# Daaohame/RAHT-3DGS-codec

Hardware: AMD Instinct MI355X
Metric: M-Gaussians/s fwd+inv RAHT, 59-ch SH3 3DGS (higher is better)
Workload: dtype f32 (xyz columns: f64); 1 GPU; cfg3: 2999072 Gaussians (3000000 draws/GPU, J=12, 59 channels), fwd RAHT + quantize/reorder + dequantize/un-reorder + inv RAHT (quantization fused into the transform kernels); the 3 xyz columns carried in float64 inside the same launches (raht_fwd_quant_mixed / raht_dequant_inv_mixed): the reference's integers on every column; rows_per_gpu=2999072, channels=59, depth_J=12, engine=tile, quantize=True, parallelism=1 GPU, world=1

## Files before the change

### raht-3dgs-codec_amd/csrc/schedule.hip

```cpp
#include "raht_common.h"

#include <algorithm>
#include <atomic>

namespace raht {

__global__ void compact_scatter_kernel(const uint32_t *in, const uint32_t *flag, const uint32_t *pos, uint32_t *out, int64_t n);

__global__ void stage_survivor_kernel(const uint32_t *__restrict__ rows, int64_t n, int R, int64_t N,
                                      const int32_t *__restrict__ wl, const int32_t *__restrict__ wr,
                                      const uint8_t *__restrict__ lvl, int top_level,
                                      uint32_t *__restrict__ survivor)
{
    const int64_t j = (int64_t)blockIdx.x * blockDim.x + threadIdx.x;
    if (j >= n) return;
    const int64_t r = rows ? rows[j] : j;
    const int64_t t = j / R;
    const int64_t j0 = t * R, j1 = j0 + R;
    const int64_t start = rows ? rows[j0] : j0;
    const int64_t end = (j1 < n) ? (rows ? (int64_t)rows[j1] : j1) : N;
    const bool merged = (r > 0) && ((int)lvl[r] < top_level) && (r - wl[r] >= start) && (r + wr[r] <= end);
    survivor[j] = merged ? 0u : 1u;
}

// ... 398 lines not shown
                                   const int64_t *__restrict__ wsum, int top_level, uint32_t *__restrict__ pj,
                                   double *__restrict__ ab, uint8_t *__restrict__ bucket, uint32_t *__restrict__ is_root)
{
    const int64_t e = (int64_t)blockIdx.x * blockDim.x + threadIdx.x;
    if (e >= n) return;
    const int64_t r = rows ? (int64_t)rows[e] : e;
    const int l = (int)lvl[r];
    const bool merged = (r > 0) && (l < top_level);
    is_root[e] = merged ? 0u : 1u;
    bucket[e] = merged ? (uint8_t)l : (uint8_t)63;
    uint32_t rec = 0;
    double a = 0.0, b = 0.0;
    if (merged) {
        const int64_t want = r - wl[r];
        int64_t p = want;
        if (rows) {
            int64_t lo = 0, hi = e - 1;
            while (lo < hi) {
                const int64_t mid = (lo + hi) >> 1;
                if ((int64_t)rows[mid] < want) lo = mid + 1; else hi = mid;
            }
            p = lo;
        }
        double w0, w1;
        pair_weights(r, wl[r], wr[r], wsum, w0, w1);
        const double den = w0 + w1;
        a = sqrt(w0 / den);
        b = sqrt(w1 / den);
        rec = (uint32_t)p | ((uint32_t)e << 16);
    }
    pj[e] = rec; ab[2 * e] = a; ab[2 * e + 1] = b;
}

__global__ void top_gather_kernel(const uint32_t *__restrict__ perm, uint32_t n_merges, const uint32_t *__restrict__ pj,
                                  const double *__restrict__ ab, uint32_t *__restrict__ t_pj,
                                  float *__restrict__ t_ab32, double *__restrict__ t_ab64)
{
    const uint32_t k = blockIdx.x * blockDim.x + threadIdx.x;
    if (k >= n_merges) return;
    const uint32_t e = perm[k];
    t_pj[k] = pj[e];
    const double a = ab[2 * e], b = ab[2 * e + 1];
    t_ab64[2 * k] = a; t_ab64[2 * k + 1] = b;
    t_ab32[2 * k] = (float)a; t_ab32[2 * k + 1] = (float)b;
}

__global__ void top_root_rank_kernel(const uint32_t *__restrict__ is_root, const uint32_t *__restrict__ pos, int64_t n,
                                     uint32_t *__restrict__ t_root)
{
    const int64_t e = (int64_t)blockIdx.x * blockDim.x + threadIdx.x;
    if (e < n) t_root[e] = is_root[e] ? pos[e] : 0xffffffffu;
}

static hipError_t gather_stage_meta(const raht_plan *plan, Stage &st, hipStream_t s)
{
    const size_t n = (size_t)st.n_entries;
    hipError_t e = hipSuccess;
    if ((e = st.e_wl.alloc(n)) != hipSuccess || (e = st.e_wr.alloc(n)) != hipSuccess || (e = st.e_lvl.alloc(n)) != hipSuccess ||
        (e = st.e_pos.alloc(n)) != hipSuccess) return e;
    hipLaunchKernelGGL(gather_meta_kernel, dim3((unsigned)ceil_div((int64_t)n, 256)), dim3(256), 0, s, st.rows, (int64_t)n, plan->wl,
                       plan->wr, plan->lvl, plan->inv_order, st.e_wl, st.e_wr, st.e_lvl, st.e_pos);
    return hipSuccess;
}

static int build_top_stage(raht_plan *plan, int64_t n, hipStream_t s, Stage &st)
{
    st.is_top = true;
    st.n_entries = n;
    st.n_tiles = 1;
    st.tile_rows = (int)n;
    const uint32_t *rows = st.rows;
    const unsigned gb = (unsigned)ceil_div(n, 256);
    if (rows) RAHT_HIP_CHECK(gather_stage_meta(plan, st, s));
    Scratch buf(sizeof(double) * 2 * (size_t)n + sizeof(uint32_t) * (4 * (size_t)n + 66) + (size_t)n, s);
    if (!buf.ok()) return RAHT_ERR_NOMEM;
    double *ab = buf.as<double>();
    uint32_t *pj = (uint32_t *)(ab + 2 * n), *is_root = pj + n, *pos = is_root + n, *perm = pos + n, *boff = perm + n,
             *total = boff + 65;
    uint8_t *bucket = (uint8_t *)(total + 1);
    hipLaunchKernelGGL(top_resolve_kernel, dim3(gb), dim3(256), 0, s, rows, n, plan->wl, plan->wr, plan->lvl, plan->wsum,
                       plan->top_level, pj, ab, bucket, is_root);
    RAHT_RET(exclusive_scan_u32(is_root, pos, n, total, s));
    RAHT_HIP_CHECK(st.t_root.alloc((size_t)n));
    hipLaunchKernelGGL(top_root_rank_kernel, dim3(gb), dim3(256), 0, s, is_root, pos, n, st.t_root);
    RAHT_RET(bucket_sort_u8(bucket, perm, n, 6, boff, s));
    RAHT_RET(read_back_u32(st.t_loff, boff, 65, nullptr, nullptr, 0, s));
    st.n_merges = st.t_loff[63];
    {
        uint32_t *lev = st.t_lev_host;
        int nlev = 0;
        for (int l = 0; l < 63; ++l)
            if (st.t_loff[l + 1] > st.t_loff[l]) { lev[2 * nlev] = st.t_loff[l]; lev[2 * nlev + 1] = st.t_loff[l + 1]; ++nlev; }
        int nbig = nlev;
        while (nbig > 0 && lev[2 * (nbig - 1) + 1] - lev[2 * (nbig - 1)] <= 64) --nbig;
        const size_t lds_budget = 160 * 1024 - 1024;
        while (nbig < nlev && (size_t)n * 16 + (size_t)(st.n_merges - lev[2 * nbig]) * 20 > lds_budget) ++nbig;
        st.t_nlev = nlev; st.t_nbig = nbig;
        st.t_small_start = (nbig < nlev) ? lev[2 * nbig] : st.n_merges;
        RAHT_HIP_CHECK(st.t_lev.alloc(2 * 64));
        RAHT_HIP_CHECK(hipMemcpyAsync(st.t_lev, lev, sizeof(uint32_t) * 2 * (size_t)std::max(nlev, 1), hipMemcpyHostToDevice, s));
    }
    const size_t nm = std::max<size_t>(st.n_merges, 1);
    RAHT_HIP_CHECK(st.t_pj.alloc(nm));
    RAHT_HIP_CHECK(st.t_ab32.alloc(2 * nm));
    RAHT_HIP_CHECK(st.t_ab64.alloc(2 * nm));
    if (st.n_merges)
        hipLaunchKernelGGL(top_gather_kernel, dim3((unsigned)ceil_div(st.n_merges, 256)), dim3(256), 0, s, perm, st.n_merges,
                           pj, ab, st.t_pj, st.t_ab32, st.t_ab64);
    return RAHT_OK;
}

constexpr int SB_THREADS = 256, SB_ITEMS = 8, SB_BLOCK = SB_THREADS * SB_ITEMS;
constexpr int SCHED_SPEC_MAX = 8;
enum { SK_NONE = 0, SK_TILE = 1, SK_TOP = 2 };

struct SchedState {
    uint32_t n[SCHED_SPEC_MAX + 2];
    uint32_t kind[SCHED_SPEC_MAX + 2];
    uint32_t finished;
    uint32_t last_stage, last_is_top;
    uint32_t trouble;
    uint32_t top[4];
};
constexpr int SCHED_STATE_WORDS = sizeof(SchedState) / 4;

__device__ __forceinline__ uint32_t block_sum_256(uint32_t v, uint32_t *red )
{
#pragma unroll
    for (int d = 32; d >= 1; d >>= 1) v += __shfl_xor(v, d, 64);
    if ((threadIdx.x & 63) == 0) red[threadIdx.x >> 6] = v;
    __syncthreads();
    const uint32_t t = red[0] + red[1] + red[2] + red[3];
    __syncthreads();
    return t;
// ... 107 lines not shown
#pragma unroll
        for (int q = 0; q < SB_ITEMS; ++q) { f[q] = (base + q < n) ? flags[base + q] : 0; mine += f[q]; }
    }
    uint32_t inc = mine;
    const int lane = threadIdx.x & 63, wid = threadIdx.x >> 6;
#pragma unroll
    for (int d = 1; d < 64; d <<= 1) { const uint32_t t = __shfl_up(inc, d, 64); if (lane >= d) inc += t; }
    if (lane == 63) wsum[wid] = inc;
    __syncthreads();
    uint32_t before = 0, block_tot = 0;
#pragma unroll
    for (int w = 0; w < 4; ++w) { if (w < wid) before += wsum[w]; block_tot += wsum[w]; }
    uint32_t pos = block_base + before + inc - mine;
    uint32_t tile = (uint32_t)base / (uint32_t)R;
    uint32_t next_start = tile * (uint32_t)R;
    if (next_start < (uint32_t)base) { ++tile; next_start += (uint32_t)R; }
    uint32_t g_r[SB_ITEMS], g_pos[SB_ITEMS], g_inv[SB_ITEMS];
    int32_t g_wl[SB_ITEMS], g_wr[SB_ITEMS];
    uint8_t g_lv[SB_ITEMS];
    bool keep[SB_ITEMS];
#pragma unroll
    for (int q = 0; q < SB_ITEMS; ++q) {
        const int64_t j = base + q;
        keep[q] = false; g_pos[q] = 0; g_r[q] = (uint32_t)j;
        if (j < n) {
            if ((uint32_t)j == next_start) { surv_off[tile] = pos; ++tile; next_start += (uint32_t)R; }
            if (f[q]) {
                keep[q] = pos < cap_next;
                g_pos[q] = pos;
                if (keep[q] && rows) g_r[q] = rows[j];
                ++pos;
            }
        }
    }
#pragma unroll
    for (int q = 0; q < SB_ITEMS; ++q) {
        g_wl[q] = 0; g_wr[q] = 0; g_lv[q] = 0; g_inv[q] = 0;
        if (keep[q]) { const uint32_t r = g_r[q]; g_wl[q] = p_wl[r]; g_wr[q] = p_wr[r]; g_lv[q] = p_lvl[r]; g_inv[q] = p_inv[r]; }
    }
#pragma unroll
    for (int q = 0; q < SB_ITEMS; ++q)
        if (keep[q]) { const uint32_t o = g_pos[q]; n_rows[o] = g_r[q]; n_wl[o] = g_wl[q]; n_wr[o] = g_wr[q]; n_lvl[o] = g_lv[q]; n_pos[o] = g_inv[q]; }
    if ((int64_t)blockIdx.x == nblk - 1 && threadIdx.x == 0) {
        const uint32_t total = block_base + block_tot;
        surv_off[(n + R - 1) / R] = total;
        S->n[k + 1] = total;
        if (total > cap_next) S->trouble = 1;
        else if (total == n_roots) { S->finished = 1; S->last_stage = (uint32_t)k; S->last_is_top = 0; }
        else if (total >= (uint32_t)n) S->trouble = 2;
        else S->kind[k + 1] = (total <= Rf) ? SK_TOP : SK_TILE;
    }
}

constexpr int ST_THREADS = 1024;
struct SchedTopOut { uint32_t *t_pj; float *t_ab32; double *t_ab64; uint32_t *t_root; uint32_t *t_lev; };

__device__ __forceinline__ void sched_top_body(SchedState *__restrict__ S, int k, int n, const uint32_t *__restrict__ rows,
                                               const int32_t *__restrict__ p_wl, const int32_t *__restrict__ p_wr,
                                               const uint8_t *__restrict__ p_lvl, const int64_t *__restrict__ wsum,
                                               int top_level, const SchedTopOut &O)
{
    __shared__ uint32_t s_rows[RAHT_TOP_MAX_ROWS];
    __shared__ uint32_t hist[64], cursor[64], wtot[ST_THREADS / 64];
    __shared__ uint32_t root_base;
    uint32_t *__restrict__ t_pj = O.t_pj, *__restrict__ t_root = O.t_root, *__restrict__ t_lev = O.t_lev;
    float *__restrict__ t_ab32 = O.t_ab32;
    double *__restrict__ t_ab64 = O.t_ab64;
    const int tid = threadIdx.x, lane = tid & 63, wid = tid >> 6;
    if (tid < 64) hist[tid] = 0;
    if (tid == 0) root_base = 0;
    for (int e = tid; e < n; e += ST_THREADS) s_rows[e] = rows ? rows[e] : (uint32_t)e;
    __syncthreads();
    PL_STAMP(2, 0, 8);
    for (int e0 = 0; e0 < n; e0 += ST_THREADS) {
        const int e = e0 + tid;
        bool root = false;
        if (e < n) {
            const uint32_t r = s_rows[e];
            const int l = (int)p_lvl[r];
            const bool merged = (r > 0) && (l < top_level);
            root = !merged;
            if (merged) atomicAdd(&hist[l], 1u);
        }
        const uint64_t bal = __ballot(root);
        if (lane == 0) wtot[wid] = (uint32_t)__popcll(bal);
        __syncthreads();
        uint32_t before = root_base;
        for (int w = 0; w < wid; ++w) before += wtot[w];
        if (e < n) t_root[e] = root ? before + (uint32_t)__popcll(bal & (((uint64_t)1 << lane) - 1)) : 0xffffffffu;
        __syncthreads();
        if (tid == 0) { uint32_t t = 0; for (int w = 0; w < ST_THREADS / 64; ++w) t += wtot[w]; root_base += t; }
        __syncthreads();
    }
    PL_STAMP(2, 0, 9);
    if (wid == 0) {
        const uint32_t h = (lane < 63) ? hist[lane] : 0u;
        uint32_t inc = h;
#pragma unroll
        for (int d = 1; d < 64; d <<= 1) { const uint32_t t = __shfl_up(inc, d, 64); if (lane >= d) inc += t; }
        const uint32_t first = inc - h;
        cursor[lane] = first;
        const uint32_t n_merges = (uint32_t)__shfl((int)inc, 63, 64);
        const uint64_t nonempty = __ballot(h > 0), below = ((uint64_t)1 << lane) - 1;
        const int nlev = __popcll(nonempty);
        const int my = __popcll(nonempty & below);
        if (h > 0) { t_lev[2 * my] = first; t_lev[2 * my + 1] = first + h; }
        const uint64_t big = __ballot(h > 64);
        int nbig = big ? __popcll(nonempty & (((uint64_t)2 << (63 - __clzll((long long)big))) - 1)) : 0;
        const size_t lds_budget = 160 * 1024 - 1024;
        uint32_t small_start = n_merges;
        for (;;) {
            uint32_t cand = n_merges;
            if (nbig < nlev) {
                const uint64_t owner = __ballot(h > 0 && my == nbig);
                cand = (uint32_t)__shfl((int)first, __ffsll((unsigned long long)owner) - 1, 64);
            }
            if (nbig < nlev && (size_t)n * 16 + (size_t)(n_merges - cand) * 20 > lds_budget) { ++nbig; continue; }
            small_start = cand;
            break;
        }
        if (lane == 0) {
            S->top[0] = n_merges; S->top[1] = (uint32_t)nlev; S->top[2] = (uint32_t)nbig; S->top[3] = small_start;
            S->finished = 1; S->last_stage = (uint32_t)k; S->last_is_top = 1;
        }
    }
    __syncthreads();
    PL_STAMP(2, 0, 10);
    for (int e = tid; e < n; e += ST_THREADS) {
        const uint32_t r = s_rows[e];
        const int l = (int)p_lvl[r];
        if (!((r > 0) && (l < top_level))) continue;
        const int32_t wlr = p_wl[r], wrr = p_wr[r];
        const uint32_t want = r - (uint32_t)wlr;
        int lo = 0, hi = e - 1;
        while (lo < hi) {
            const int mid = (lo + hi) >> 1;
            if (s_rows[mid] < want) lo = mid + 1; else hi = mid;
        }
        double w0, w1;
        pair_weights((int64_t)r, wlr, wrr, wsum, w0, w1);
        const double den = w0 + w1;
        const double a = sqrt(w0 / den), b = sqrt(w1 / den);
        const uint32_t pos = atomicAdd(&cursor[l], 1u);
        t_pj[pos] = (uint32_t)lo | ((uint32_t)e << 16);
        t_ab64[2 * pos] = a; t_ab64[2 * pos + 1] = b;
        t_ab32[2 * pos] = (float)a; t_ab32[2 * pos + 1] = (float)b;
    }
    PL_STAMP(2, 0, 11);
}

struct SchedStageBufs {
    uint32_t *rows[SCHED_SPEC_MAX + 2]; int32_t *wl[SCHED_SPEC_MAX + 2], *wr[SCHED_SPEC_MAX + 2];
    uint8_t *lvl[SCHED_SPEC_MAX + 2]; uint32_t *pos[SCHED_SPEC_MAX + 2], *surv[SCHED_SPEC_MAX + 2];
    uint32_t cap[SCHED_SPEC_MAX + 2];
};

__global__ __launch_bounds__(ST_THREADS) void sched_tail_kernel(SchedState *S, int k_multi, int k_last, SchedStageBufs B, int R, uint32_t Rf,
                                                                uint32_t n_roots, int64_t N, int top_level, uint32_t tail_max,
                                                                const int32_t *__restrict__ p_wl, const int32_t *__restrict__ p_wr,
                                                                const uint8_t *__restrict__ p_lvl, const uint32_t *__restrict__ p_inv,
                                                                const int64_t *__restrict__ wsum, SchedTopOut O, int64_t n_first)
{
    __shared__ uint32_t wcnt[8 * (ST_THREADS / 64)], woff[8 * (ST_THREADS / 64) + 1];
    __shared__ uint32_t s_kind[SCHED_SPEC_MAX + 2], s_n[SCHED_SPEC_MAX + 2];
    const int tid = threadIdx.x, lane = tid & 63, wid = tid >> 6;
    PL_SLOT_DECL;
    PL_STAMP_NEXT();
    if (n_first >= 0) { sched_state_init(S, (uint32_t)n_first, SK_TOP); __builtin_amdgcn_fence(__ATOMIC_RELEASE, "workgroup"); __syncthreads(); }
    if (tid < SCHED_SPEC_MAX + 2) {
        s_kind[tid] = (n_first >= 0) ? (tid == 0 ? (uint32_t)SK_TOP : (uint32_t)SK_NONE) : __atomic_load_n(&S->kind[tid], __ATOMIC_RELAXED);
        s_n[tid] = (n_first >= 0) ? (tid == 0 ? (uint32_t)n_first : 0u) : __atomic_load_n(&S->n[tid], __ATOMIC_RELAXED);
    }
    __syncthreads();
    for (int k = (k_multi == 0) ? 0 : 1; k <= k_last; ++k) {
        const uint32_t kind = s_kind[k], n = s_n[k];
        PL_STAMP_NEXT();
        if (kind == SK_TOP) {
            sched_top_body(S, k, (int)n, B.rows[k], p_wl, p_wr, p_lvl, wsum, top_level, O);
            return;
        }
        if (kind == SK_TILE && k < k_multi) continue;
        if (kind != SK_TILE || n > tail_max || n > B.cap[k] || k == k_last) return;
        const uint32_t *__restrict__ rows = B.rows[k];
        const int32_t *__restrict__ wl = B.wl[k], *__restrict__ wr = B.wr[k];
        const uint8_t *__restrict__ lvl = B.lvl[k];
        uint32_t *__restrict__ surv_off = B.surv[k];
        uint32_t *__restrict__ n_rows = B.rows[k + 1], *__restrict__ n_pos = B.pos[k + 1];
        int32_t *__restrict__ n_wl = B.wl[k + 1], *__restrict__ n_wr = B.wr[k + 1];
        uint8_t *__restrict__ n_lvl = B.lvl[k + 1];
        const uint32_t cap_next = B.cap[k + 1];
        uint32_t running = 0;
        constexpr int TI = 8, NWV = ST_THREADS / 64;
        for (uint32_t base = 0; base < n; base += ST_THREADS * TI) {
            uint32_t r[TI], e_start[TI], e_end[TI];
            int32_t e_wl[TI], e_wr[TI];
            uint8_t e_lv[TI];
            uint64_t bal[TI];
// ... 293 lines not shown
```

### raht-3dgs-codec_amd/csrc/transform_mx.hip

```cpp
#include "raht_common.h"
#include "raht_device.h"
#include "tile_engine.h"
#include "tile_host.h"

#include <algorithm>
#include <cstdlib>
#include <string>
#include <type_traits>
#include <vector>

namespace raht {

#ifdef RAHT_PHASE_CLOCKS
constexpr int MX_CLK_TILES = 4096, MX_CLK_SLOTS = 12;
__device__ unsigned long long g_phase_clk_mx[MX_CLK_TILES][MX_CLK_SLOTS];
#define MX_STAMP(k) do { if (IDENT && threadIdx.x == 0 && tile_id < MX_CLK_TILES) g_phase_clk_mx[tile_id][k] = __builtin_readcyclecounter(); } while (0)
#else
#define MX_STAMP(k) do { } while (0)
#endif

constexpr int MX_MAX_WIDE = 4;
constexpr int MX_THREADS = 512;
constexpr int MX_TOP_THREADS = 1024;
constexpr int MX_TOP_SLOTS = RAHT_TOP_MAX_ROWS / MX_TOP_THREADS;

struct StepTableMX {
    StepTable f;
    double w[MX_MAX_WIDE];
};

static size_t tile_lds_bytes_mx(int R, int NF, int nwide)
{
    const size_t data = (size_t)R * NF * 16 + (((size_t)R * nwide * 8 + 15) & ~(size_t)15);
    const size_t meta = (size_t)R * (16 + 4 + 4);
    const size_t surv = ((size_t)R * 2 + 15) & ~(size_t)15;
    return data + meta + surv;
}

struct MxPtrs {
    const double *in_w;
    double *out_w;
    double *wsn_w;
    double *root_w;
    const uint32_t *prog;
    uint32_t prog_stride, prog_ab;
    int prog_compact;
};

struct MxMultiQ {
    int k;
    uint32_t fast_div;
    double step[MULTI_Q_MAX];
    int32_t *Q[MULTI_Q_MAX];
};

template <bool INV, bool IDENT, int SLOTS, bool ROOTS, bool MULTI = false, bool SQ = false>
__device__ __forceinline__ void tile_body_mx(const TileArgs<float> &A, const MxPtrs &P, const StepTableMX &ST, const int64_t tile_id,
                                             const MxMultiQ *MQ = nullptr)
{
    extern __shared__ __align__(16) unsigned char smem[];
    typedef RegChunk<float> V16;
    typedef RegChunk<double> W16;
    typedef RegChunk<int32_t> I16;
    const int R = A.R;
    const int tid0 = threadIdx.x;
    const int nthreads = blockDim.x, nwv = nthreads >> 6;
    const int nwide = A.nwide;
    const int lgw = nwide > 2 ? 2 : nwide - 1;
    const int Df = A.D;
    const int Fp = A.Dp, NF = Fp >> 2;
    const int lg = A.lg, lr = 6 - A.lg;
// ... 533 lines not shown
__global__ __launch_bounds__(MX_THREADS, 6) void tile_kernel_mx_sq(const TileArgs<float> A, const MxPtrs P, const StepTableMX ST)
{
    tile_body_mx<true, true, SLOTS, false, false, true>(A, P, ST, (int64_t)blockIdx.x);
}

struct TileBatchMX {
    TileArgs<float> a[BATCH_MAX];
    MxPtrs p[BATCH_MAX];
    uint32_t first_tile[BATCH_MAX + 1];
    int n;
};
static_assert(sizeof(TileBatchMX) + sizeof(StepTableMX) <= 4096, "tile_kernel_mx_batch: arguments exceed the 4 KB kernarg segment");

template <bool INV, bool IDENT, int SLOTS>
__global__ __launch_bounds__(MX_THREADS, 6) void tile_kernel_mx_batch(const TileBatchMX B, const StepTableMX ST)
{
    int s = 0;
#pragma unroll
    for (int q = 1; q < BATCH_MAX; ++q) s += (q < B.n && blockIdx.x >= B.first_tile[q]) ? 1 : 0;
    tile_body_mx<INV, IDENT, SLOTS, false>(B.a[s], B.p[s], ST, (int64_t)(blockIdx.x - B.first_tile[s]));
}

struct TopArgsMX {
    const float *in_rows;  int64_t ld_in;
    const float *in_img; const double *in_img_w;
    float *out_rows;       int64_t ld_out;
    float *out_img; double *out_img_w;
    int32_t *Q;            int64_t ldq;
    const uint32_t *e_pos;
    const uint32_t *pj;
    const float *ab32;  const double *ab64;
    int n, n_merges, D, nwide, Fp;
    const uint32_t *lev;
    int nlev, nbig;
    uint32_t small_start;
    const uint32_t *root_rank;
    float *root_f; double *root_w;
};

template <bool WIDE, bool INV, bool ROOTS, bool MULTI = false>
__device__ __forceinline__ void top_body_mx(const TopArgsMX &A, const StepTableMX &ST, const int chunk, const MxMultiQ *MQ = nullptr)
{
    typedef typename std::conditional<WIDE, double, float>::type T;
    constexpr int VN = WIDE ? 2 : 4;
    typedef RegChunk<T> V16;
    extern __shared__ __align__(16) unsigned char smem[];
    V16 *tile = (V16 *)smem;
    __shared__ uint32_t s_lev[2 * 64];
    const int tid = threadIdx.x;
    const int nwide = A.nwide;
    const int goff = WIDE ? 2 * chunk : min(chunk * 4, A.D - 4);
    const int ioff = chunk * 4;
    const int n = A.n, nm = A.n_merges;
    if (tid < 2 * A.nlev) s_lev[tid] = A.lev[tid];
    const T *ab = WIDE ? (const T *)A.ab64 : (const T *)A.ab32;
    const int n_small = nm - (int)A.small_start;
    uint32_t *s_pj = (uint32_t *)(smem + (size_t)n * 16);
    T *s_ab = (T *)(s_pj + ((n_small + 3) & ~3));
    for (int i = tid; i < n_small; i += MX_TOP_THREADS) {
        s_pj[i] = A.pj[A.small_start + i];
        s_ab[2 * i] = ab[2 * (A.small_start + i)];
        s_ab[2 * i + 1] = ab[2 * (A.small_start + i) + 1];
    }
    T my_step[VN];
    float my_rcp[VN];
    bool live[VN];
#pragma unroll
    for (int i = 0; i < VN; ++i) {
        if constexpr (WIDE) { live[i] = goff + i < nwide; my_step[i] = live[i] ? ST.w[goff + i] : 1.0; my_rcp[i] = 1.0f; }
        else { live[i] = !(chunk == 0 && i < nwide); my_step[i] = ST.f.v[ST.f.n == 1 ? 0 : goff + i]; my_rcp[i] = refined_rcp(my_step[i]); }
    }
    uint32_t pj[MX_TOP_SLOTS];
    T ra[MX_TOP_SLOTS], rb[MX_TOP_SLOTS];
#pragma unroll
    for (int k = 0; k < MX_TOP_SLOTS; ++k) {
        const int idx = min(k * MX_TOP_THREADS + tid, max(nm - 1, 0));
        pj[k] = A.pj[idx]; ra[k] = ab[2 * idx]; rb[k] = ab[2 * idx + 1];
    }
    uint32_t m_dst[MX_TOP_SLOTS], m_rr[MX_TOP_SLOTS];
#pragma unroll
    for (int k = 0; k < MX_TOP_SLOTS; ++k) {
        m_dst[k] = A.e_pos[min(k * MX_TOP_THREADS + tid, n - 1)];
        m_rr[k] = ROOTS ? A.root_rank[min(k * MX_TOP_THREADS + tid, n - 1)] : 0xffffffffu;
    }
#pragma unroll
    for (int k = 0; k < MX_TOP_SLOTS; ++k) {
        const int e = k * MX_TOP_THREADS + tid;
        if (e >= n) continue;
        V16 v;
        if constexpr (!INV) {
            if (A.in_img) {
                if constexpr (WIDE) {
#pragma unroll
                    for (int i = 0; i < VN; ++i) v.v[i] = live[i] ? A.in_img_w[(int64_t)e * nwide + goff + i] : 0.0;
                } else {
                    v = *(const V16 *)(A.in_img + (int64_t)e * A.Fp + ioff);
                }
            } else if constexpr (WIDE) {
#pragma unroll
                for (int i = 0; i < VN; ++i) v.v[i] = live[i] ? (double)A.in_rows[(int64_t)e * A.ld_in + goff + i] : 0.0;
            } else {
                v = ld_chunk<float>(A.in_rows + (int64_t)e * A.ld_in + goff);
            }
        } else if (m_rr[k] != 0xffffffffu) {
            if constexpr (WIDE) {
#pragma unroll
                for (int i = 0; i < VN; ++i) v.v[i] = live[i] ? A.root_w[(int64_t)m_rr[k] * nwide + goff + i] : 0.0;
            } else {
                v = ld_chunk<float>(A.root_f + (int64_t)m_rr[k] * A.D + goff);
            }
        } else {
            const int32_t *q = A.Q + (int64_t)m_dst[k] * A.ldq + goff;
            if constexpr (WIDE) {
#pragma unroll
                for (int i = 0; i < VN; ++i) v.v[i] = live[i] ? (double)q[i] * my_step[i] : 0.0;
            } else {
                const RegChunk<int32_t> raw = ld_chunk<int32_t>(q);
#pragma unroll
                for (int i = 0; i < VN; ++i) v.v[i] = (float)raw.v[i] * my_step[i];
            }
        }
        tile[e] = v;
    }
    __syncthreads();

    auto butterfly = [&](uint32_t rec, T a, T b) {
        const uint32_t ip = rec & 0xffffu, ij = rec >> 16;
        const V16 x0 = tile[ip], x1 = tile[ij];
        V16 vlo, vhi;
#pragma unroll
        for (int i = 0; i < VN; ++i) {
            if (!INV) {
                vlo.v[i] = a * x0.v[i] + b * x1.v[i];
                vhi.v[i] = a * x1.v[i] - b * x0.v[i];
            } else {
                vlo.v[i] = a * x0.v[i] - b * x1.v[i];
                vhi.v[i] = b * x0.v[i] + a * x1.v[i];
            }
        }
        tile[ip] = vlo; tile[ij] = vhi;
    };
    auto big_levels = [&]() {
#pragma unroll 1
        for (int q = 0; q < A.nbig; ++q) {
            const int li = INV ? A.nbig - 1 - q : q;
            const uint32_t lo = s_lev[2 * li], hi = s_lev[2 * li + 1];
#pragma unroll
            for (int k = 0; k < MX_TOP_SLOTS; ++k) {
                const uint32_t idx = (uint32_t)(k * MX_TOP_THREADS + tid);
                if ((uint32_t)(k * MX_TOP_THREADS) < hi && (uint32_t)((k + 1) * MX_TOP_THREADS) > lo && idx >= lo && idx < hi)
                    butterfly(pj[k], ra[k], rb[k]);
            }
            __syncthreads();
        }
    };
    auto small_levels = [&]() {
        if (tid < 64) {
#pragma unroll 1
            for (int q = A.nbig; q < A.nlev; ++q) {
                const int li = INV ? A.nlev - 1 - (q - A.nbig) : q;
                const uint32_t lo = s_lev[2 * li], hi = s_lev[2 * li + 1];
                const uint32_t i = lo - A.small_start + (uint32_t)tid;
                if (lo + (uint32_t)tid < hi) butterfly(s_pj[i], s_ab[2 * i], s_ab[2 * i + 1]);
            }
        }
        __syncthreads();
    };
    if (!INV) { big_levels(); small_levels(); }
    else { small_levels(); big_levels(); }

#pragma unroll
    for (int k = 0; k < MX_TOP_SLOTS; ++k) {
        const int e = k * MX_TOP_THREADS + tid;
        if (e >= n) continue;
        const V16 v = tile[e];
        if constexpr (INV) {
            if (A.out_img) {
                if constexpr (WIDE) {
#pragma unroll
                    for (int i = 0; i < VN; ++i) if (live[i]) A.out_img_w[(int64_t)e * nwide + goff + i] = v.v[i];
                } else {
                    *(V16 *)(A.out_img + (int64_t)e * A.Fp + ioff) = v;
                }
            } else if constexpr (WIDE) {
#pragma unroll
                for (int i = 0; i < VN; ++i) if (live[i]) A.out_rows[(int64_t)e * A.ld_out + goff + i] = (float)v.v[i];
            } else if (chunk == 0) {
#pragma unroll
                for (int i = 0; i < VN; ++i) if (live[i]) A.out_rows[(int64_t)e * A.ld_out + goff + i] = v.v[i];
            } else {
                st_chunk<float>(A.out_rows + (int64_t)e * A.ld_out + goff, v);
            }
        } else if (m_rr[k] != 0xffffffffu) {
            if constexpr (WIDE) {
#pragma unroll
                for (int i = 0; i < VN; ++i) if (live[i]) A.root_w[(int64_t)m_rr[k] * nwide + goff + i] = v.v[i];
            } else {
                st_chunk<float>(A.root_f + (int64_t)m_rr[k] * A.D + goff, v);
            }
        } else if constexpr (MULTI) {
            for (int kk = 0; kk < MQ->k; ++kk) {
                int32_t *q = MQ->Q[kk] + (int64_t)m_dst[k] * A.ldq + goff;
                if constexpr (WIDE) {
#pragma unroll
                    for (int i = 0; i < VN; ++i) if (live[i]) q[i] = quantize_one_f64(v.v[i], MQ->step[kk]);
                } else {
                    const float sf = (float)MQ->step[kk], rf = refined_rcp(sf);
                    const int fd = (int)((MQ->fast_div >> kk) & 1u);
                    RegChunk<int32_t> qv;
#pragma unroll
                    for (int i = 0; i < VN; ++i) qv.v[i] = quantize_one(v.v[i], sf, rf, fd);
                    if (chunk == 0) {
#pragma unroll
                        for (int i = 0; i < VN; ++i) if (live[i]) q[i] = qv.v[i];
                    } else {
                        st_chunk<int32_t>(q, qv);
                    }
                }
            }
        } else {
            int32_t *q = A.Q + (int64_t)m_dst[k] * A.ldq + goff;
            if constexpr (WIDE) {
#pragma unroll
                for (int i = 0; i < VN; ++i) if (live[i]) q[i] = quantize_one_f64(v.v[i], my_step[i]);
            } else {
                RegChunk<int32_t> qv;
#pragma unroll
                for (int i = 0; i < VN; ++i) qv.v[i] = quantize_one(v.v[i], my_step[i], my_rcp[i], ST.f.fast_div);
                if (chunk == 0) {
#pragma unroll
                    for (int i = 0; i < VN; ++i) if (live[i]) q[i] = qv.v[i];
                } else {
                    st_chunk<int32_t>(q, qv);
                }
            }
        }
    }
}

template <bool INV>
__global__ __launch_bounds__(MX_TOP_THREADS) void top_kernel_mx(const TopArgsMX A, const StepTableMX ST)
{
    const int NW2 = (A.nwide + 1) >> 1;
    if ((int)blockIdx.x < NW2) top_body_mx<true, INV, false>(A, ST, (int)blockIdx.x);
    else top_body_mx<false, INV, false>(A, ST, (int)blockIdx.x - NW2);
}
template <bool INV>
__global__ __launch_bounds__(MX_TOP_THREADS) void top_kernel_mx_roots(const TopArgsMX A, const StepTableMX ST)
{
    const int NW2 = (A.nwide + 1) >> 1;
    if ((int)blockIdx.x < NW2) top_body_mx<true, INV, true>(A, ST, (int)blockIdx.x);
    else top_body_mx<false, INV, true>(A, ST, (int)blockIdx.x - NW2);
}

struct TopBatchMX { TopArgsMX a[BATCH_MAX]; };
static_assert(sizeof(TopBatchMX) + sizeof(StepTableMX) <= 4096, "top_kernel_mx_batch: arguments exceed the 4 KB kernarg segment");

template <bool INV>
__global__ __launch_bounds__(MX_TOP_THREADS) void top_kernel_mx_batch(const TopBatchMX B, const StepTableMX ST)
{
    const TopArgsMX &A = B.a[blockIdx.y];
    const int NW2 = (A.nwide + 1) >> 1;
    if ((int)blockIdx.x < NW2) top_body_mx<true, INV, false>(A, ST, (int)blockIdx.x);
    else top_body_mx<false, INV, false>(A, ST, (int)blockIdx.x - NW2);
}

__global__ __launch_bounds__(MX_TOP_THREADS) void top_kernel_mx_multi(const TopArgsMX A, const StepTableMX ST, const MxMultiQ M)
{
    const int NW2 = (A.nwide + 1) >> 1;
    if ((int)blockIdx.x < NW2) top_body_mx<true, false, false, true>(A, ST, (int)blockIdx.x, &M);
    else top_body_mx<false, false, false, true>(A, ST, (int)blockIdx.x - NW2, &M);
}

__global__ void mx_cols_to_f64_kernel(const float *__restrict__ C, int64_t ldc, int64_t N, int nwide, double *__restrict__ W)
{
    const int64_t e = (int64_t)blockIdx.x * blockDim.x + threadIdx.x;
    if (e >= N * nwide) return;
    const int64_t i = e / nwide;
    W[e] = (double)C[i * ldc + (e - i * nwide)];
}
__global__ void mx_cols_from_f64_kernel(const double *__restrict__ W, int64_t N, int nwide, float *__restrict__ C, int64_t ldc)
{
    const int64_t e = (int64_t)blockIdx.x * blockDim.x + threadIdx.x;
    if (e >= N * nwide) return;
    const int64_t i = e / nwide;
    C[i * ldc + (e - i * nwide)] = (float)W[e];
}

struct MxGeom {
    int nwide = 0, NCp = 0, Dp = 0, lg = 0;
// ... 553 lines not shown

int raht_fwd_quant_mixed_multi(const raht_plan *plan, const float *C, int64_t ldc, int D, const double *steps, int k, int n_wide,
                               int32_t *const *Q, int64_t ldq, raht_stream_t stream)
{
    return guarded("raht_fwd_quant_mixed_multi", [&]() { return fwd_quant_mixed_multi_impl(plan, C, ldc, D, steps, k, n_wide, Q, ldq, stream); });
}

int raht_dequant_inv_mixed_sqdiff(const raht_plan *plan, const int32_t *Q, int64_t ldq, int D, const double *steps, int n_steps,
                                  int n_wide, const float *C_ref, int64_t ld_ref, float *C_rec, int64_t ldc, double *sqdiff,
                                  raht_stream_t stream)
{
    return guarded("raht_dequant_inv_mixed_sqdiff", [&]() {
        return dequant_inv_mixed_sqdiff_impl(plan, Q, ldq, D, steps, n_steps, n_wide, C_ref, ld_ref, C_rec, ldc, sqdiff, stream); });
}

int raht_fwd_quant_mixed_batch(int n, raht_plan *const *plans, const float *const *C, const int64_t *ldc, int D,
                               const double *steps, int n_steps, int n_wide, int32_t *const *Q, const int64_t *ldq, raht_stream_t stream)
{
    const char *what = "raht_fwd_quant_mixed_batch";
    return guarded(what, [&]() -> int {
        RAHT_RET(mx_batch_check_args(what, n, plans, (const void *const *)C, ldc, (const void *const *)Q, ldq, D, steps, n_steps, n_wide));
        std::vector<MxIO> ios((size_t)n);
        for (int i = 0; i < n; ++i) { MxIO &io = ios[(size_t)i]; io.C_in = C[i]; io.ldc = ldc[i]; io.Q = Q[i]; io.ldq = ldq[i]; }
        return run_batch_mx<false>(what, n, plans, ios.data(), D, steps, n_steps, n_wide, (hipStream_t)stream);
    });
}

int raht_dequant_inv_mixed_batch(int n, raht_plan *const *plans, const int32_t *const *Q, const int64_t *ldq, int D,
                                 const double *steps, int n_steps, int n_wide, float *const *C, const int64_t *ldc, raht_stream_t stream)
{
    const char *what = "raht_dequant_inv_mixed_batch";
    return guarded(what, [&]() -> int {
        RAHT_RET(mx_batch_check_args(what, n, plans, (const void *const *)Q, ldq, (const void *const *)C, ldc, D, steps, n_steps, n_wide));
        std::vector<MxIO> ios((size_t)n);
        for (int i = 0; i < n; ++i) { MxIO &io = ios[(size_t)i]; io.C_out = C[i]; io.ldc = ldc[i]; io.Q = const_cast<int32_t *>(Q[i]); io.ldq = ldq[i]; }
        return run_batch_mx<true>(what, n, plans, ios.data(), D, steps, n_steps, n_wide, (hipStream_t)stream);
    });
}

int raht_mixed_batch_stats(int n, raht_plan *const *plans, int D, int n_wide, int inverse, int *tile_launches, int *top_launches,
                           int *single_scene_calls)
{
    return guarded("raht_mixed_batch_stats", [&]() {
        return mixed_batch_stats_impl(n, plans, D, n_wide, inverse, tile_launches, top_launches, single_scene_calls); });
}

#ifdef RAHT_PHASE_CLOCKS
int raht_debug_read_phase_clocks_mx(unsigned long long *dst, int n_tiles)
{
    RAHT_HIP_CHECK(hipDeviceSynchronize());
    RAHT_HIP_CHECK(hipMemcpyFromSymbol(dst, HIP_SYMBOL(g_phase_clk_mx), sizeof(unsigned long long) * MX_CLK_SLOTS * (size_t)std::min(n_tiles, MX_CLK_TILES)));
    return MX_CLK_SLOTS;
}
#endif

int raht_plan_mixed_stats(raht_plan *plan, int D, int n_wide, int *tile_rows, int *n_stages, int64_t *rows_per_stage, int max_stages)
{
    return guarded("raht_plan_mixed_stats", [&]() -> int {
        if (!plan || !tile_rows || !n_stages || D < 1 || n_wide < 1 || n_wide > MX_MAX_WIDE) { set_error("raht_plan_mixed_stats: bad argument"); return RAHT_ERR_INVALID; }
        RAHT_RET(check_plan_device(plan, "raht_plan_mixed_stats"));
        *tile_rows = 0; *n_stages = 0;
        if (plan->row_map) return RAHT_OK;
        Schedule *sc = nullptr;
        MxGeom g;
        RAHT_RET(mx_setup(plan, D, n_wide, D, nullptr, &sc, g));
        if (!sc) return RAHT_OK;
        *tile_rows = g.R0;
        *n_stages = (int)sc->stages.size();
        for (int k = 0; k < *n_stages && k < max_stages && rows_per_stage; ++k) rows_per_stage[k] = sc->stages[(size_t)k].n_entries;
        return RAHT_OK;
    });
}

}
```

Baseline: 5026 M-Gaussians/s.

## Bucket top-stage merges by dependency height and pipeline top-kernel loads

Top-stage merges are now bucketed by dependency height, computed by a shared-memory level sweep, instead of by tree level. This can collapse the number of serial butterfly levels in the top kernel. The top kernel's load phase is restructured to issue all input, metadata and merge-record loads up front into registers, with compiler pins, before writing to LDS. The small-level loop now prefetches the next level's record while processing the current one. It adds more register pressure and complexity, and optional debug clock stamps.

Measured after the change: 5005 M-Gaussians/s. No clear change (-0.4%).

```diff
diff --git a/raht-3dgs-codec_amd/csrc/schedule.hip b/raht-3dgs-codec_amd/csrc/schedule.hip
--- a/raht-3dgs-codec_amd/csrc/schedule.hip
+++ b/raht-3dgs-codec_amd/csrc/schedule.hip
@@ -474,6 +474,51 @@
     if (e < n) t_root[e] = is_root[e] ? pos[e] : 0xffffffffu;
 }
 
+constexpr int ST_THREADS = 1024;
+constexpr int TOP_HT_SLOTS = RAHT_TOP_MAX_ROWS / ST_THREADS;
+
+__device__ __forceinline__ void top_heights(uint8_t *cur, const uint32_t *present, const uint32_t (&mg)[TOP_HT_SLOTS], int n, int tid)
+{
+#pragma unroll
+    for (int q = 0; q < TOP_HT_SLOTS; ++q) if (q * ST_THREADS + tid < n) cur[q * ST_THREADS + tid] = 0;
+    __syncthreads();
+    for (uint64_t m = (uint64_t)present[0] | ((uint64_t)present[1] << 32); m; m &= m - 1) {
+        const int l = __ffsll((unsigned long long)m) - 1;
+#pragma unroll
+        for (int q = 0; q < TOP_HT_SLOTS; ++q) {
+            if ((int)(mg[q] >> 16) != l + 1) continue;
+            const int e = q * ST_THREADS + tid, p = (int)(mg[q] & 0xffffu);
+            const uint8_t h = (uint8_t)(1 + max((int)cur[p], (int)cur[e]));
+            cur[p] = h; cur[e] = h;
+        }
+        __syncthreads();
+    }
+}
+
+__global__ __launch_bounds__(ST_THREADS) void top_heights_kernel(const uint32_t *__restrict__ pj, uint8_t *__restrict__ bucket, int n)
+{
+    __shared__ uint8_t s_cur[RAHT_TOP_MAX_ROWS];
+    __shared__ uint32_t present[2];
+    const int tid = threadIdx.x;
+    if (tid < 2) present[tid] = 0;
+    __syncthreads();
+    uint32_t mg[TOP_HT_SLOTS];
+#pragma unroll
+    for (int q = 0; q < TOP_HT_SLOTS; ++q) {
+        const int e = q * ST_THREADS + tid;
+        mg[q] = 0;
+        if (e < n && bucket[e] != 63) {
+            const uint32_t l = bucket[e];
+            mg[q] = ((l + 1) << 16) | (pj[e] & 0xffffu);
+            atomicOr(&present[l >> 5], 1u << (l & 31));
+        }
+    }
+    __syncthreads();
+    top_heights(s_cur, present, mg, n, tid);
+#pragma unroll
+    for (int q = 0; q < TOP_HT_SLOTS; ++q) if (mg[q]) bucket[q * ST_THREADS + tid] = (uint8_t)(s_cur[q * ST_THREADS + tid] - 1);
+}
+
 static hipError_t gather_stage_meta(const raht_plan *plan, Stage &st, hipStream_t s)
 {
     const size_t n = (size_t)st.n_entries;
@@ -487,6 +532,7 @@
 
 static int build_top_stage(raht_plan *plan, int64_t n, hipStream_t s, Stage &st)
 {
+    if (n > RAHT_TOP_MAX_ROWS) { set_error("top stage: %lld entries (at most %d)", (long long)n, RAHT_TOP_MAX_ROWS); return RAHT_ERR_INVALID; }
     st.is_top = true;
     st.n_entries = n;
     st.n_tiles = 1;
@@ -502,6 +548,7 @@
     uint8_t *bucket = (uint8_t *)(total + 1);
     hipLaunchKernelGGL(top_resolve_kernel, dim3(gb), dim3(256), 0, s, rows, n, plan->wl, plan->wr, plan->lvl, plan->wsum,
                        plan->top_level, pj, ab, bucket, is_root);
+    hipLaunchKernelGGL(top_heights_kernel, dim3(1), dim3(ST_THREADS), 0, s, pj, bucket, (int)n);
     RAHT_RET(exclusive_scan_u32(is_root, pos, n, total, s));
     RAHT_HIP_CHECK(st.t_root.alloc((size_t)n));
     hipLaunchKernelGGL(top_root_rank_kernel, dim3(gb), dim3(256), 0, s, is_root, pos, n, st.t_root);
@@ -715,7 +762,6 @@
     }
 }
 
-constexpr int ST_THREADS = 1024;
 struct SchedTopOut { uint32_t *t_pj; float *t_ab32; double *t_ab64; uint32_t *t_root; uint32_t *t_lev; };
 
 __device__ __forceinline__ void sched_top_body(SchedState *__restrict__ S, int k, int n, const uint32_t *__restrict__ rows,
@@ -724,13 +770,16 @@
                                                int top_level, const SchedTopOut &O)
 {
     __shared__ uint32_t s_rows[RAHT_TOP_MAX_ROWS];
-    __shared__ uint32_t hist[64], cursor[64], wtot[ST_THREADS / 64];
+    __shared__ uint16_t s_part[RAHT_TOP_MAX_ROWS];
+    __shared__ uint8_t s_cur[RAHT_TOP_MAX_ROWS];
+    __shared__ uint32_t hist[64], cursor[64], wtot[ST_THREADS / 64], present[2];
     __shared__ uint32_t root_base;
     uint32_t *__restrict__ t_pj = O.t_pj, *__restrict__ t_root = O.t_root, *__restrict__ t_lev = O.t_lev;
     float *__restrict__ t_ab32 = O.t_ab32;
     double *__restrict__ t_ab64 = O.t_ab64;
     const int tid = threadIdx.x, lane = tid & 63, wid = tid >> 6;
     if (tid < 64) hist[tid] = 0;
+    if (tid < 2) present[tid] = 0;
     if (tid == 0) root_base = 0;
     for (int e = tid; e < n; e += ST_THREADS) s_rows[e] = rows ? rows[e] : (uint32_t)e;
     __syncthreads();
@@ -743,7 +792,6 @@
             const int l = (int)p_lvl[r];
             const bool merged = (r > 0) && (l < top_level);
             root = !merged;
-            if (merged) atomicAdd(&hist[l], 1u);
         }
         const uint64_t bal = __ballot(root);
         if (lane == 0) wtot[wid] = (uint32_t)__popcll(bal);
@@ -755,6 +803,32 @@
         if (tid == 0) { uint32_t t = 0; for (int w = 0; w < ST_THREADS / 64; ++w) t += wtot[w]; root_base += t; }
         __syncthreads();
     }
+    for (int e = tid; e < n; e += ST_THREADS) {
+        const uint32_t r = s_rows[e];
+        const int l = (int)p_lvl[r];
+        s_cur[e] = 0xff;
+        if (!((r > 0) && (l < top_level))) continue;
+        const uint32_t want = r - (uint32_t)p_wl[r];
+        int lo = 0, hi = e - 1;
+        while (lo < hi) {
+            const int mid = (lo + hi) >> 1;
+            if (s_rows[mid] < want) lo = mid + 1; else hi = mid;
+        }
+        s_part[e] = (uint16_t)lo; s_cur[e] = (uint8_t)l;
+        atomicOr(&present[l >> 5], 1u << (l & 31));
+    }
+    __syncthreads();
+    uint32_t mg[TOP_HT_SLOTS];
+#pragma unroll
+    for (int q = 0; q < TOP_HT_SLOTS; ++q) {
+        const int e = q * ST_THREADS + tid;
+        mg[q] = (e < n && s_cur[e] != 0xff) ? (((uint32_t)s_cur[e] + 1) << 16) | (uint32_t)s_part[e] : 0u;
+    }
+    __syncthreads();
+    top_heights(s_cur, present, mg, n, tid);
+#pragma unroll
+    for (int q = 0; q < TOP_HT_SLOTS; ++q) if (mg[q]) atomicAdd(&hist[s_cur[q * ST_THREADS + tid] - 1], 1u);
+    __syncthreads();
     PL_STAMP(2, 0, 9);
     if (wid == 0) {
         const uint32_t h = (lane < 63) ? hist[lane] : 0u;
@@ -794,18 +868,12 @@
         const int l = (int)p_lvl[r];
         if (!((r > 0) && (l < top_level))) continue;
         const int32_t wlr = p_wl[r], wrr = p_wr[r];
-        const uint32_t want = r - (uint32_t)wlr;
-        int lo = 0, hi = e - 1;
-        while (lo < hi) {
-            const int mid = (lo + hi) >> 1;
-            if (s_rows[mid] < want) lo = mid + 1; else hi = mid;
-        }
         double w0, w1;
         pair_weights((int64_t)r, wlr, wrr, wsum, w0, w1);
         const double den = w0 + w1;
         const double a = sqrt(w0 / den), b = sqrt(w1 / den);
-        const uint32_t pos = atomicAdd(&cursor[l], 1u);
-        t_pj[pos] = (uint32_t)lo | ((uint32_t)e << 16);
+        const uint32_t pos = atomicAdd(&cursor[s_cur[e] - 1], 1u);
+        t_pj[pos] = (uint32_t)s_part[e] | ((uint32_t)e << 16);
         t_ab64[2 * pos] = a; t_ab64[2 * pos + 1] = b;
         t_ab32[2 * pos] = (float)a; t_ab32[2 * pos + 1] = (float)b;
     }
diff --git a/raht-3dgs-codec_amd/csrc/transform_mx.hip b/raht-3dgs-codec_amd/csrc/transform_mx.hip
--- a/raht-3dgs-codec_amd/csrc/transform_mx.hip
+++ b/raht-3dgs-codec_amd/csrc/transform_mx.hip
@@ -15,8 +15,12 @@
 constexpr int MX_CLK_TILES = 4096, MX_CLK_SLOTS = 12;
 __device__ unsigned long long g_phase_clk_mx[MX_CLK_TILES][MX_CLK_SLOTS];
 #define MX_STAMP(k) do { if (IDENT && threadIdx.x == 0 && tile_id < MX_CLK_TILES) g_phase_clk_mx[tile_id][k] = __builtin_readcyclecounter(); } while (0)
+constexpr int MX_TOP_CLK_SLOTS = 6;
+__device__ unsigned long long g_top_clk_mx[2][2][MX_TOP_CLK_SLOTS];
+#define TOP_STAMP(k) do { if (chunk == 0 && threadIdx.x == 0) g_top_clk_mx[INV ? 1 : 0][WIDE ? 1 : 0][k] = __builtin_readcyclecounter(); } while (0)
 #else
 #define MX_STAMP(k) do { } while (0)
+#define TOP_STAMP(k) do { } while (0)
 #endif
 
 constexpr int MX_MAX_WIDE = 4;
@@ -656,16 +660,11 @@
     const int goff = WIDE ? 2 * chunk : min(chunk * 4, A.D - 4);
     const int ioff = chunk * 4;
     const int n = A.n, nm = A.n_merges;
-    if (tid < 2 * A.nlev) s_lev[tid] = A.lev[tid];
     const T *ab = WIDE ? (const T *)A.ab64 : (const T *)A.ab32;
-    const int n_small = nm - (int)A.small_start;
+    const int small_start = (int)A.small_start, n_small = nm - small_start;
     uint32_t *s_pj = (uint32_t *)(smem + (size_t)n * 16);
     T *s_ab = (T *)(s_pj + ((n_small + 3) & ~3));
-    for (int i = tid; i < n_small; i += MX_TOP_THREADS) {
-        s_pj[i] = A.pj[A.small_start + i];
-        s_ab[2 * i] = ab[2 * (A.small_start + i)];
-        s_ab[2 * i + 1] = ab[2 * (A.small_start + i) + 1];
-    }
+    TOP_STAMP(0);
     T my_step[VN];
     float my_rcp[VN];
     bool live[VN];
@@ -674,59 +673,133 @@
         if constexpr (WIDE) { live[i] = goff + i < nwide; my_step[i] = live[i] ? ST.w[goff + i] : 1.0; my_rcp[i] = 1.0f; }
         else { live[i] = !(chunk == 0 && i < nwide); my_step[i] = ST.f.v[ST.f.n == 1 ? 0 : goff + i]; my_rcp[i] = refined_rcp(my_step[i]); }
     }
-    uint32_t pj[MX_TOP_SLOTS];
-    T ra[MX_TOP_SLOTS], rb[MX_TOP_SLOTS];
-#pragma unroll
-    for (int k = 0; k < MX_TOP_SLOTS; ++k) {
+    constexpr int S = MX_TOP_SLOTS;
+    uint32_t m_dst[S], m_rr[S], pj[S];
+    T ra[S], rb[S];
+    auto load_phase = [&](auto ns, auto kb) {
+    constexpr int NS = decltype(ns)::value, KB = decltype(kb)::value;
+    uint32_t raw_[NS][4];
+    uint32_t (*raw)[4] = raw_ - KB;
+    asm volatile("" ::: "memory");
+    auto pin_u32 = [](uint32_t (&x)[S]) {
+        if constexpr (NS == 4) asm volatile("" : "+v"(x[KB + 3]), "+v"(x[KB + 2]), "+v"(x[KB + 1]), "+v"(x[KB]) :: "memory");
+        else if constexpr (NS == 2) asm volatile("" : "+v"(x[KB + 1]), "+v"(x[KB]) :: "memory");
+        else asm volatile("" : "+v"(x[KB]) :: "memory");
+    };
+#pragma unroll
+    for (int k = KB; k < KB + NS; ++k) {
+        const int ec = min(k * MX_TOP_THREADS + tid, n - 1);
+        m_dst[k] = A.e_pos[ec];
+        m_rr[k] = ROOTS ? A.root_rank[ec] : 0xffffffffu;
+    }
+    uint32_t levv = A.lev[min(tid, max(2 * A.nlev - 1, 0))];
+#pragma unroll
+    for (int k = KB; k < KB + NS; ++k) {
         const int idx = min(k * MX_TOP_THREADS + tid, max(nm - 1, 0));
         pj[k] = A.pj[idx]; ra[k] = ab[2 * idx]; rb[k] = ab[2 * idx + 1];
     }
-    uint32_t m_dst[MX_TOP_SLOTS], m_rr[MX_TOP_SLOTS];
-#pragma unroll
-    for (int k = 0; k < MX_TOP_SLOTS; ++k) {
-        m_dst[k] = A.e_pos[min(k * MX_TOP_THREADS + tid, n - 1)];
-        m_rr[k] = ROOTS ? A.root_rank[min(k * MX_TOP_THREADS + tid, n - 1)] : 0xffffffffu;
-    }
-#pragma unroll
-    for (int k = 0; k < MX_TOP_SLOTS; ++k) {
+    if constexpr (INV) {
+        if constexpr (ROOTS) pin_u32(m_rr);
+        pin_u32(m_dst);
+    }
+    const int c0 = WIDE ? goff : 0, c1 = WIDE ? min(goff + 1, nwide - 1) : 0;
+    struct __attribute__((packed, aligned(4))) U2 { uint32_t a, b; };
+#pragma unroll
+    for (int k = KB; k < KB + NS; ++k) {
+        {
+            const int64_t e = min(k * MX_TOP_THREADS + tid, n - 1);
+            if constexpr (!INV) {
+                if constexpr (WIDE) {
+                    const char *base = A.in_img ? (const char *)A.in_img_w : (const char *)A.in_rows;
+                    const int64_t ld = A.in_img ? (int64_t)nwide * 8 : A.ld_in * 4;
+                    const int esz = A.in_img ? 8 : 4;
+                    const U2 lo = *(const U2 *)(base + e * ld + c0 * esz), hi = *(const U2 *)(base + e * ld + c1 * esz);
+                    raw[k][0] = lo.a; raw[k][1] = lo.b; raw[k][2] = hi.a; raw[k][3] = hi.b;
+                } else {
+                    const float *src = A.in_img ? A.in_img + ioff : A.in_rows + goff;
+                    const RegChunk<float> t = ld_chunk<float>(src + e * (A.in_img ? (int64_t)A.Fp : A.ld_in));
+#pragma unroll
+                    for (int i = 0; i < 4; ++i) raw[k][i] = __float_as_uint(t.v[i]);
+                }
+            } else {
+                const bool is_root = ROOTS && m_rr[k] != 0xffffffffu;
+                const int32_t *q = A.Q + (int64_t)m_dst[k] * A.ldq;
+                if constexpr (WIDE && ROOTS) {
+                    const double *rw = A.root_w + (int64_t)(is_root ? m_rr[k] : 0u) * nwide;
+                    const U2 lo = *(is_root ? (const U2 *)(rw + c0) : (const U2 *)(q + c0));
+                    const U2 hi = *(is_root ? (const U2 *)(rw + c1) : (const U2 *)(q + c1));
+                    raw[k][0] = lo.a; raw[k][1] = lo.b; raw[k][2] = hi.a; raw[k][3] = hi.b;
+                } else if constexpr (WIDE) {
+                    raw[k][0] = (uint32_t)q[c0]; raw[k][1] = (uint32_t)q[c1];
+                    raw[k][2] = raw[k][3] = 0;
+                } else {
+                    const int32_t *p = is_root ? (const int32_t *)(A.root_f + (int64_t)m_rr[k] * A.D + goff) : q + goff;
+                    const RegChunk<int32_t> t = ld_chunk<int32_t>(p);
+#pragma unroll
+                    for (int i = 0; i < 4; ++i) raw[k][i] = (uint32_t)t.v[i];
+                }
+            }
+        }
+    }
+    TOP_STAMP(1);
+#pragma unroll
+    for (int k = KB + NS - 1; k >= KB; --k) asm volatile("" : "+v"(raw[k][0]), "+v"(raw[k][1]), "+v"(raw[k][2]), "+v"(raw[k][3]) :: "memory");
+    pin_u32(pj);
+    if constexpr (!INV) { if constexpr (ROOTS) pin_u32(m_rr); pin_u32(m_dst); }
+    asm volatile("" : "+v"(levv) :: "memory");
+    if (tid < 2 * A.nlev) s_lev[tid] = levv;
+#pragma unroll
+    for (int k = KB; k < KB + NS; ++k) {
+        const int i = k * MX_TOP_THREADS + tid - small_start;
+        if (i >= 0 && i < n_small) { s_pj[i] = pj[k]; s_ab[2 * i] = ra[k]; s_ab[2 * i + 1] = rb[k]; }
+    }
+#pragma unroll
+    for (int k = KB; k < KB + NS; ++k) {
         const int e = k * MX_TOP_THREADS + tid;
         if (e >= n) continue;
         V16 v;
         if constexpr (!INV) {
-            if (A.in_img) {
+            if constexpr (WIDE) {
+#pragma unroll
+                for (int i = 0; i < VN; ++i) {
+                    const double x = A.in_img ? __hiloint2double((int)raw[k][2 * i + 1], (int)raw[k][2 * i]) : (double)__uint_as_float(raw[k][2 * i]);
+                    v.v[i] = live[i] ? x : 0.0;
+                }
+            } else {
+#pragma unroll
+                for (int i = 0; i < VN; ++i) v.v[i] = __uint_as_float(raw[k][i]);
+            }
+        } else {
+            const bool is_root = ROOTS && m_rr[k] != 0xffffffffu;
+#pragma unroll
+            for (int i = 0; i < VN; ++i) {
                 if constexpr (WIDE) {
-#pragma unroll
-                    for (int i = 0; i < VN; ++i) v.v[i] = live[i] ? A.in_img_w[(int64_t)e * nwide + goff + i] : 0.0;
+                    const double r = __hiloint2double((int)raw[k][2 * i + 1], (int)raw[k][2 * i]);
+                    const double x = is_root ? r : (double)(int32_t)raw[k][ROOTS ? 2 * i : i] * my_step[i];
+                    v.v[i] = live[i] ? x : 0.0;
                 } else {
-                    v = *(const V16 *)(A.in_img + (int64_t)e * A.Fp + ioff);
-                }
-            } else if constexpr (WIDE) {
-#pragma unroll
-                for (int i = 0; i < VN; ++i) v.v[i] = live[i] ? (double)A.in_rows[(int64_t)e * A.ld_in + goff + i] : 0.0;
-            } else {
-                v = ld_chunk<float>(A.in_rows + (int64_t)e * A.ld_in + goff);
-            }
-        } else if (m_rr[k] != 0xffffffffu) {
-            if constexpr (WIDE) {
-#pragma unroll
-                for (int i = 0; i < VN; ++i) v.v[i] = live[i] ? A.root_w[(int64_t)m_rr[k] * nwide + goff + i] : 0.0;
-            } else {
-                v = ld_chunk<float>(A.root_f + (int64_t)m_rr[k] * A.D + goff);
-            }
-        } else {
-            const int32_t *q = A.Q + (int64_t)m_dst[k] * A.ldq + goff;
-            if constexpr (WIDE) {
-#pragma unroll
-                for (int i = 0; i < VN; ++i) v.v[i] = live[i] ? (double)q[i] * my_step[i] : 0.0;
-            } else {
-                const RegChunk<int32_t> raw = ld_chunk<int32_t>(q);
-#pragma unroll
-                for (int i = 0; i < VN; ++i) v.v[i] = (float)raw.v[i] * my_step[i];
+                    v.v[i] = is_root ? __uint_as_float(raw[k][i]) : (float)(int32_t)raw[k][i] * my_step[i];
+                }
             }
         }
         tile[e] = v;
     }
     __syncthreads();
+    pin_u32(m_dst); pin_u32(pj);
+    if constexpr (ROOTS) pin_u32(m_rr);
+#pragma unroll
+    for (int k = KB; k < KB + NS; ++k) asm volatile("" : "+v"(ra[k]), "+v"(rb[k]));
+#pragma unroll
+    for (int k = KB + NS; k < S; ++k) { m_dst[k] = 0; m_rr[k] = 0xffffffffu; pj[k] = 0; ra[k] = T(0); rb[k] = T(0); }
+    };
+    typedef std::integral_constant<int, 0> K0;
+    if (n <= MX_TOP_THREADS) load_phase(std::integral_constant<int, 1>(), K0());
+    else if (n <= 2 * MX_TOP_THREADS) load_phase(std::integral_constant<int, 2>(), K0());
+    else {
+        load_phase(std::integral_constant<int, 4>(), K0());
+        if (n > 4 * MX_TOP_THREADS) load_phase(std::integral_constant<int, 4>(), std::integral_constant<int, 4>());
+    }
+    TOP_STAMP(2);
 
     auto butterfly = [&](uint32_t rec, T a, T b) {
         const uint32_t ip = rec & 0xffffu, ij = rec >> 16;
@@ -760,18 +833,31 @@
     };
     auto small_levels = [&]() {
         if (tid < 64) {
+            const int nch = A.nlev - A.nbig;
+            uint32_t my_lo = 0, my_hi = 0;
+            if (tid < nch) {
+                const int li = INV ? A.nlev - 1 - tid : A.nbig + tid;
+                my_lo = s_lev[2 * li]; my_hi = s_lev[2 * li + 1];
+            }
+            uint32_t rec = 0; T ra_n = T(0), rb_n = T(0); bool on_n = false;
+            auto fetch = [&](int q) {
+                const uint32_t lo = (uint32_t)__builtin_amdgcn_readlane((int)my_lo, q), hi = (uint32_t)__builtin_amdgcn_readlane((int)my_hi, q);
+                const uint32_t i = min(lo - (uint32_t)small_start + (uint32_t)tid, (uint32_t)max(n_small - 1, 0));
+                on_n = lo + (uint32_t)tid < hi;
+                rec = s_pj[i]; ra_n = s_ab[2 * i]; rb_n = s_ab[2 * i + 1];
+            };
+            if (nch > 0) fetch(0);
 #pragma unroll 1
-            for (int q = A.nbig; q < A.nlev; ++q) {
-                const int li = INV ? A.nlev - 1 - (q - A.nbig) : q;
-                const uint32_t lo = s_lev[2 * li], hi = s_lev[2 * li + 1];
-                const uint32_t i = lo - A.small_start + (uint32_t)tid;
-                if (lo + (uint32_t)tid < hi) butterfly(s_pj[i], s_ab[2 * i], s_ab[2 * i + 1]);
+            for (int q = 0; q < nch; ++q) {
+                const uint32_t rec_c = rec; const T ra_c = ra_n, rb_c = rb_n; const bool on_c = on_n;
+                if (q + 1 < nch) fetch(q + 1);
+                if (on_c) butterfly(rec_c, ra_c, rb_c);
             }
         }
         __syncthreads();
     };
-    if (!INV) { big_levels(); small_levels(); }
-    else { small_levels(); big_levels(); }
+    if (!INV) { big_levels(); TOP_STAMP(3); small_levels(); TOP_STAMP(4); }
+    else { small_levels(); TOP_STAMP(3); big_levels(); TOP_STAMP(4); }
 
 #pragma unroll
     for (int k = 0; k < MX_TOP_SLOTS; ++k) {
@@ -840,6 +926,7 @@
             }
         }
     }
+    TOP_STAMP(5);
 }
 
 template <bool INV>
@@ -1499,6 +1586,12 @@
     RAHT_HIP_CHECK(hipMemcpyFromSymbol(dst, HIP_SYMBOL(g_phase_clk_mx), sizeof(unsigned long long) * MX_CLK_SLOTS * (size_t)std::min(n_tiles, MX_CLK_TILES)));
     return MX_CLK_SLOTS;
 }
+int raht_debug_read_top_clocks_mx(unsigned long long *dst)
+{
+    RAHT_HIP_CHECK(hipDeviceSynchronize());
+    RAHT_HIP_CHECK(hipMemcpyFromSymbol(dst, HIP_SYMBOL(g_top_clk_mx), sizeof(unsigned long long) * 4 * MX_TOP_CLK_SLOTS));
+    return MX_TOP_CLK_SLOTS;
+}
 #endif
 
 int raht_plan_mixed_stats(raht_plan *plan, int D, int n_wide, int *tile_rows, int *n_stages, int64_t *rows_per_stage, int max_stages)
```
